# arcosoph/nanowakeword

Measured on AMD Instinct MI355X. Metric: clips/sec (1 s @16 kHz PCM->logits), higher is better.
Workload: dtype f32; 1 GPU; cnn head on (101,64) log-mel, batch=4096/GPU, 1 s 16 kHz mono int16 clips, 64-mel 25 ms/10 ms center frontend, fused STFT+mel HIP kernel, fp32; clips_per_gpu=4096, n_samples=16000, parallelism=batch-split x1

## Files before the change

### nanowakeword_amd/build.py

```python
from __future__ import annotations

import os
import shutil
import subprocess
import sys

PKG = os.path.dirname(os.path.abspath(__file__))
ROOT = os.path.dirname(PKG)
CSRC = os.path.join(PKG, "csrc")
LIB = os.path.join(PKG, "libnwwhip.so")
EMU_DIR = os.path.join(ROOT, "tests", "hostemu")
EMU_LIB = os.path.join(EMU_DIR, "libfe_emu.so")

HIP_SOURCES = ["nww_api.hip", "nww_weights.hip", "nww_plan.hip", "nww_stream.hip", "nww_comm.hip", "nww_emb.hip", "frontend2.hip", "layers.hip", "gemm_x3.hip", "trunk.hip", "trunk_b.hip", "conv3_x3.hip", "ffn_x3.hip", "lin_x3.hip", "dual_x3.hip", "bc_chain.hip", "rnn_x3.hip", "rnn_stream.hip", "mha_mfma.hip", "mha_h2.hip", "attn_x3.hip", "emb_stream.hip", "tcn_x3.hip", "merge_x3.hip", "qn_x3.hip", "raw_conv.hip", "raw_x3.hip", "fe_tables.cpp"]


def _hipcc() -> str:
    for c in (os.environ.get("HIPCC"), shutil.which("hipcc"), "/opt/rocm/bin/hipcc"):
        if c and os.path.exists(c):
            return c
    raise RuntimeError("hipcc not found")


def _newer(target: str, deps) -> bool:
    if not os.path.exists(target):
        return True
    t = os.path.getmtime(target)
    return any(os.path.getmtime(d) > t for d in deps)


NO_SLP = {"frontend2.hip", "trunk_b.hip", "dual_x3.hip", "bc_chain.hip", "layers.hip", "ffn_x3.hip"}


def build_hip(force: bool = False, verbose: bool = False, out: str = LIB) -> str:
    from concurrent.futures import ThreadPoolExecutor
    tag = "" if out == LIB else "_" + os.path.splitext(os.path.basename(out))[0]
    odir = os.path.join(PKG, "build" + tag)
    os.makedirs(odir, exist_ok=True)
    mode = os.environ.get("NWW_SLP", "")
    extra = os.environ.get("NWW_HIPCC_FLAGS", "").split()
    headers = [os.path.join(CSRC, f) for f in os.listdir(CSRC) if f.endswith(".h")] + [os.path.join(ROOT, "include", "nww.h")]
    jobs, objs = [], []
    for src in HIP_SOURCES:
        sp = os.path.join(CSRC, src)
        obj = os.path.join(odir, os.path.splitext(src)[0] + ".o")
        objs.append(obj)
        if not force and not _newer(obj, [sp] + headers):
            continue
        no_slp = mode == "none" or (mode != "all" and src in NO_SLP)
        jobs.append([_hipcc(), "--offload-arch=gfx950", "-O3", "-std=c++17", "-fPIC"] + (["-fno-slp-vectorize"] if no_slp else []) + extra +
                    ["-I", CSRC, "-I", os.path.join(ROOT, "include"), "-x", "hip", "-c", sp, "-o", obj])
    if not jobs and os.path.exists(out) and not _newer(out, objs):
        return out

    def run(cmd):
        if verbose:
            print(" ".join(cmd), flush=True)
        subprocess.run(cmd, check=True)
    with ThreadPoolExecutor(max_workers=max(1, int(os.environ.get("NWW_BUILD_JOBS", "6")))) as ex:
        list(ex.map(run, jobs))
    subprocess.run([_hipcc(), "--offload-arch=gfx950", "-shared", "-fPIC", "-o", out] + objs, check=True)
    return out


def build_emu(force: bool = False) -> str:
    srcs = [os.path.join(EMU_DIR, "fe_emu.cpp"), os.path.join(CSRC, "fe_tables.cpp")]
    deps = srcs + [os.path.join(CSRC, "fe_steps.h"), os.path.join(CSRC, "fe_tables.h")]
    if not force and not _newer(EMU_LIB, deps):
        return EMU_LIB
    subprocess.run(["g++", "-O2", "-std=c++17", "-shared", "-fPIC", "-I", CSRC, "-o", EMU_LIB] + srcs, check=True)
    return EMU_LIB


if __name__ == "__main__":
    print(build_hip(force="--force" in sys.argv, verbose=True))
    print(build_emu(force="--force" in sys.argv))
```

### nanowakeword_amd/csrc/fe_steps.h

```cpp
#pragma once
#include <math.h>
#include <stdint.h>

#if defined(__HIPCC__)
#include <hip/hip_runtime.h>
#define NWW_HD __host__ __device__ __forceinline__
typedef float2 nww_c32;
#else
#define NWW_HD inline
struct nww_c32 { float x, y; };
#endif

#define FE_NFFT 400
#define FE_M 200
#define FE_BINS 201
#define FE_PSTRIDE 209
#define FE_MAX_MELS 128
#define FE_MAX_MELW 640

NWW_HD nww_c32 c_make(float x, float y) { nww_c32 r; r.x = x; r.y = y; return r; }
NWW_HD nww_c32 c_add(nww_c32 a, nww_c32 b) { return c_make(a.x + b.x, a.y + b.y); }
NWW_HD nww_c32 c_sub(nww_c32 a, nww_c32 b) { return c_make(a.x - b.x, a.y - b.y); }
NWW_HD nww_c32 c_mul(nww_c32 a, nww_c32 b) { return c_make(a.x * b.x - a.y * b.y, a.x * b.y + a.y * b.x); }
NWW_HD nww_c32 c_mul_negi(nww_c32 a) { return c_make(a.y, -a.x); }
// ... 69 lines not shown
    for (int b = 0; b < 5; ++b) {
        if (SEQ) NWW_SCHED_FENCE();
        dft5(u[b][0], u[b][1], u[b][2], u[b][3], u[b][4]);
        if (b > 0) {
#pragma unroll
            for (int c = 1; c < 5; ++c) u[b][c] = c_mul(u[b][c], w25(b * c));
        }
    }
#pragma unroll
    for (int c = 0; c < 5; ++c) {
        if (SEQ) NWW_SCHED_FENCE();
        dft5(u[0][c], u[1][c], u[2][c], u[3][c], u[4][c]);
#pragma unroll
        for (int d = 0; d < 5; ++d) store(c + 5 * d, u[d][c]);
    }
    if (SEQ) NWW_SCHED_FENCE();
}

NWW_HD void fe_s1(int f, int n2, int hop, const int16_t* span, const FeTables* tb, nww_c32* yz) {
    const uint32_t* fr = (const uint32_t*)(span + hop * f);
    nww_c32 z[8];
#pragma unroll
    for (int n1 = 0; n1 < 8; ++n1) {
        const int m = 25 * n1 + n2;
        const nww_c32 w = tb->win2[m];
        const uint32_t v = fr[m];
        z[n1] = c_make((float)(int16_t)(v & 0xffffu) * w.x, (float)(int16_t)(v >> 16) * w.y);
    }
    dft8(z);
    nww_c32* out = yz + (f * 8) * 25 + n2;
    out[0] = z[0];
#pragma unroll
    for (int k1 = 1; k1 < 8; ++k1) out[k1 * 25] = c_mul(z[k1], tb->tw200[k1 * 25 + n2]);
}

NWW_HD void fe_s2(int f, int k1, nww_c32* yz) {
    nww_c32* row = yz + (f * 8 + k1) * 25;
    dft25([&](int i) { return row[i]; }, [&](int i, nww_c32 v) { row[i] = v; });
}

NWW_HD void fe_s3_core(nww_c32 A, nww_c32 B, nww_c32 tw, float* pa, float* pb) {
    const nww_c32 E = c_make(A.x + B.x, A.y - B.y);
    const nww_c32 O = c_make(A.y + B.y, B.x - A.x);
    const nww_c32 wO = c_mul(tw, O);
    const nww_c32 Xa = c_add(E, wO), Xb = c_sub(E, wO);
    *pa = Xa.x * Xa.x + Xa.y * Xa.y;
    *pb = Xb.x * Xb.x + Xb.y * Xb.y;
}
NWW_HD int fe_zpos(int k) { return (k & 7) * 25 + (k >> 3); }

NWW_HD void fe_s3(int f, int k, const FeTables* tb, const nww_c32* yz, float* pw) {
    const nww_c32* zf = yz + f * 200;
    const int kb = (k == 0) ? 0 : 200 - k;
    float* p = pw + f * FE_PSTRIDE;
    fe_s3_core(zf[fe_zpos(k)], zf[fe_zpos(kb)], tb->tw400[k], &p[k], &p[200 - k]);
}

NWW_HD float fe_s4(int f, int j, const FeTables* tb, const float* pw) {
    const float* p = pw + f * FE_PSTRIDE + tb->mel_lo[j];
    const float* w = tb->melw + tb->mel_off[j];
    const int n = tb->mel_cnt[j];
    float acc = 0.0f;
    for (int i = 0; i < n; ++i) acc = fmaf(p[i], w[i], acc);
    return acc;
}

NWW_HD float fe_db(float mel, float amin, float mult) {
    return mult * log10f(fmaxf(mel, amin));
}

NWW_HD int fe_reflect(int s, int N) {
    if (s < 0) s = -s;
    if (s >= N) s = 2 * (N - 1) - s;
    return s;
}

#define FE2_G 8
#define FE2_FRAME_DW 400
#define FE2_PSHIFT(f) (4 * ((f) >> 1))
#define FE2_STAGE_OFF 216
#define FE2_MAX_TILES 8
#define FE2_MAX_STEPS 512

#define FE2_CHUNK 8
#define FE2_MAX_CHUNKS 64
struct Fe2MelPlan {
    int32_t ntiles;
    int32_t total_steps;
    int32_t nchunks;
    int32_t tile_k0[FE2_MAX_TILES];
    int32_t tile_nsteps[FE2_MAX_TILES];
    int32_t tile_first[FE2_MAX_TILES];
    uint32_t chunk_meta[FE2_MAX_CHUNKS];
    float b[FE2_MAX_STEPS * 64];
};

NWW_HD void fe2_s1(const uint32_t s[8], const nww_c32 win[8], const nww_c32 tw[7], nww_c32 z[8]) {
#pragma unroll
    for (int n1 = 0; n1 < 8; ++n1)
        z[n1] = c_make((float)(int16_t)(s[n1] & 0xffffu) * win[n1].x, (float)(int16_t)(s[n1] >> 16) * win[n1].y);
    dft8(z);
#pragma unroll
    for (int k1 = 1; k1 < 8; ++k1) z[k1] = c_mul(z[k1], tw[k1 - 1]);
}

NWW_HD float fe2_mel_planned(const Fe2MelPlan* pl, const float* p, int j) {
    const int t = j >> 4, n = j & 15;
    const int k0 = pl->tile_k0[t], ns = pl->tile_nsteps[t];
    const float* b = pl->b + (size_t)pl->tile_first[t] * 64 + n;
    float acc[2] = {0.0f, 0.0f};
    for (int s = 0; s < ns; ++s)
        for (int kk = 0; kk < 4; ++kk) acc[s & 1] = fmaf(p[k0 + 4 * s + kk], b[s * 64 + kk * 16], acc[s & 1]);
    return acc[0] + acc[1];
}
```

### nanowakeword_amd/csrc/fe_tables.cpp

```cpp
#include "fe_tables.h"
#include <cmath>
#include <cstring>

static const double kPi = 3.14159265358979323846;

void fe_default_window(int win_length, std::vector<float>& window) {
    window.resize(win_length);
    for (int n = 0; n < win_length; ++n)
        window[n] = (float)(0.5 - 0.5 * std::cos(2.0 * kPi * n / win_length));
}

void fe_default_melfb(const FeParams& p, std::vector<float>& fb) {
    const int n_freqs = p.n_fft / 2 + 1;
    fb.assign((size_t)n_freqs * p.n_mels, 0.f);
    const double m_min = 2595.0 * std::log10(1.0 + (double)p.f_min / 700.0);
    const double m_max = 2595.0 * std::log10(1.0 + (double)p.f_max / 700.0);
    std::vector<double> f_pts(p.n_mels + 2);
    for (int i = 0; i < p.n_mels + 2; ++i) {
        const double m = m_min + (m_max - m_min) * i / (p.n_mels + 1);
        f_pts[i] = 700.0 * (std::pow(10.0, m / 2595.0) - 1.0);
    }
    const double nyq = (double)(p.sample_rate / 2);
    for (int k = 0; k < n_freqs; ++k) {
        const double f = nyq * k / (n_freqs - 1);
// ... 6 lines not shown
    }
}

std::string fe_build_tables(const FeParams& p, const float* window, const float* fb, FeTables* t) {
    if (p.n_fft != FE_NFFT) return "only n_fft=400 is implemented";
    if (p.win_length > p.n_fft || p.win_length <= 0) return "win_length must be in 1..n_fft";
    if (p.n_mels <= 0 || p.n_mels > FE_MAX_MELS) return "n_mels must be in 1..128";
    if (p.hop <= 0 || (p.hop & 1)) return "hop_length must be positive and even";
    std::memset(t, 0, sizeof(*t));
    std::vector<float> wp(p.n_fft, 0.f);
    const int pad_left = (p.n_fft - p.win_length) / 2;
    for (int i = 0; i < p.win_length; ++i) wp[pad_left + i] = window[i];
    for (int m = 0; m < FE_M; ++m) {
        t->win2[m].x = wp[2 * m] * (1.0f / 65536.0f);
        t->win2[m].y = wp[2 * m + 1] * (1.0f / 65536.0f);
    }
    for (int n2 = 0; n2 < 25; ++n2)
        for (int k1 = 0; k1 < 8; ++k1) {
            const double a = -2.0 * kPi * (double)(n2 * k1) / 200.0;
            t->tw200[k1 * 25 + n2].x = (float)std::cos(a);
            t->tw200[k1 * 25 + n2].y = (float)std::sin(a);
        }
    for (int k = 0; k <= 100; ++k) {
        const double a = -2.0 * kPi * (double)k / 400.0;
        t->tw400[k].x = (float)std::cos(a);
        t->tw400[k].y = (float)std::sin(a);
    }
    int off = 0;
    for (int j = 0; j < p.n_mels; ++j) {
        int lo = -1, hi = -1;
        for (int k = 0; k < FE_BINS; ++k)
            if (fb[(size_t)k * p.n_mels + j] != 0.f) { if (lo < 0) lo = k; hi = k; }
        if (lo < 0) { lo = 0; hi = -1; }
        const int cnt = hi - lo + 1;
        if (off + cnt > FE_MAX_MELW) return "mel filterbank has too many non-zeros for the LDS table";
        t->mel_lo[j] = lo; t->mel_cnt[j] = cnt; t->mel_off[j] = off;
        for (int i = 0; i < cnt; ++i) t->melw[off + i] = fb[(size_t)(lo + i) * p.n_mels + j];
        off += cnt;
    }
    return "";
}

int fe_num_frames(const FeParams& p, int n) {
    if (p.center) {
        if (n <= p.n_fft / 2) return -1;
        return 1 + n / p.hop;
    }
    if (n < p.n_fft) return -1;
    return 1 + (n - p.n_fft) / p.hop;
}

std::string fe2_build_mel_plan(const FeParams& p, const float* fb, Fe2MelPlan* pl) {
    std::memset(pl, 0, sizeof(*pl));
    const int ntiles = (p.n_mels + 15) / 16;
    if (ntiles > FE2_MAX_TILES) return "n_mels must be <= 128";
    pl->ntiles = ntiles;
    int first = 0;
    for (int t = 0; t < ntiles; ++t) {
        int lo = FE_BINS, hi = -1;
        for (int k = 0; k < FE_BINS; ++k)
            for (int n = 0; n < 16; ++n) {
                const int j = 16 * t + n;
                if (j < p.n_mels && fb[(size_t)k * p.n_mels + j] != 0.f) { if (k < lo) lo = k; if (k > hi) hi = k; }
            }
        if (hi < 0) { lo = 0; hi = 0; }
        int ns = (hi - lo + 1 + 3) / 4;
        ns = (ns + FE2_CHUNK - 1) / FE2_CHUNK * FE2_CHUNK;
        if (first + ns > FE2_MAX_STEPS || (first + ns) / FE2_CHUNK > FE2_MAX_CHUNKS) return "mel filterbank is too dense for the MFMA plan";
        for (int c = 0; c < ns / FE2_CHUNK; ++c)
            pl->chunk_meta[first / FE2_CHUNK + c] =
                (uint32_t)(lo + 4 * FE2_CHUNK * c) | ((uint32_t)t << 12) | ((c == ns / FE2_CHUNK - 1) ? 1u << 16 : 0u);
        pl->tile_k0[t] = lo; pl->tile_nsteps[t] = ns; pl->tile_first[t] = first;
        for (int s = 0; s < ns; ++s)
            for (int l = 0; l < 64; ++l) {
                const int k = lo + 4 * s + (l >> 4), j = 16 * t + (l & 15);
                pl->b[(size_t)(first + s) * 64 + l] = (k < FE_BINS && j < p.n_mels) ? fb[(size_t)k * p.n_mels + j] : 0.f;
            }
        first += ns;
    }
    pl->total_steps = first;
    pl->nchunks = first / FE2_CHUNK;
    return "";
}
```

### nanowakeword_amd/csrc/fe_tables.h

```cpp
#pragma once
#include <string>
#include <vector>
#include "fe_steps.h"

struct FeParams {
    int sample_rate = 16000, n_fft = 400, win_length = 400, hop = 160, n_mels = 64, center = 1;
    float f_min = 0.f, f_max = 8000.f, amin = 1e-10f, db_mult = 10.f;
};

void fe_default_window(int win_length, std::vector<float>& window);
void fe_default_melfb(const FeParams& p, std::vector<float>& fb);

std::string fe_build_tables(const FeParams& p, const float* window, const float* fb, FeTables* out);

std::string fe2_build_mel_plan(const FeParams& p, const float* fb, Fe2MelPlan* out);

int fe_num_frames(const FeParams& p, int n_samples);
```

### nanowakeword_amd/csrc/frontend2.hip

```cpp
#include <hip/hip_runtime.h>
#include <stdlib.h>
#include "fe_steps.h"
#include "frontend.h"
#include "layers.h"

typedef float f32x4 __attribute__((ext_vector_type(4)));

struct Fe2MelLds {
    uint32_t desc[FE_MAX_MELS];
    float w[FE_MAX_MELW];
};

__device__ __forceinline__ void fe2_wave_sync() {
    __builtin_amdgcn_fence(__ATOMIC_RELEASE, "wavefront");
    __builtin_amdgcn_wave_barrier();
    __builtin_amdgcn_fence(__ATOMIC_ACQUIRE, "wavefront");
}

__device__ __forceinline__ void fe2_load_column(const int16_t* __restrict__ x, int base, int n2, uint32_t v[8]) {
    const uint32_t* p = reinterpret_cast<const uint32_t*>(x + base) + n2;
#pragma unroll
    for (int n1 = 0; n1 < 8; ++n1) v[n1] = p[25 * n1];
}

__device__ __forceinline__ float fe2_db(float mel, float amin, float mult, float floor_db) {
    const float db = (mult * 0.30102999566398120f) * __log2f(fmaxf(mel, amin));
    return mel > amin ? db : floor_db;
}

#define FE2_PARAMS                                                                                                      \
    const int16_t *__restrict__ pcm, size_t row_stride, int B, int N, int T, int ngroups, int hop, int pad, int n_mels,    \
        float amin, float db_mult, float floor_db, const FeTables *__restrict__ gtb, const Fe2MelPlan *__restrict__ plan,  \
        float *__restrict__ out_db, float *__restrict__ out_mel, int frames_major, int dbg, int gsz, Fe2Sub sub
#define FE2_ARGS pcm, row_stride, B, N, T, ngroups, hop, pad, n_mels, amin, db_mult, floor_db, gtb, plan, out_db, out_mel, frames_major, dbg, gsz, sub
template <int MEL, int FAST_OUT, int MAXT, bool RING, bool FLAT>
__device__ __forceinline__ void fe2_wave_body(FE2_PARAMS) {
    static_assert(!FLAT || (FAST_OUT && !RING && MEL == 2), "flat items: frames-major fast output, register filters, no frame subsets");
#ifndef NWW_ABLATION
    if (FLAT) dbg = 0;
#endif
    extern __shared__ __attribute__((aligned(16))) char smem[];
    constexpr int MFMA_MEL = MEL == 1;
    const int lane = threadIdx.x & 63;
    const int wv = __builtin_amdgcn_readfirstlane((int)(threadIdx.x >> 6));
    const int nwv = blockDim.x >> 6;
    const int tb_bytes = MEL == 0 ? (int)sizeof(Fe2MelLds) : 0;
    Fe2MelLds* mt = reinterpret_cast<Fe2MelLds*>(smem);
    float* slab = reinterpret_cast<float*>(smem + tb_bytes) + wv * (FE2_G * FE2_FRAME_DW);
    if (MEL == 0) {
        for (int i = threadIdx.x; i < FE_MAX_MELS; i += blockDim.x)
            mt->desc[i] = (uint32_t)gtb->mel_lo[i] | ((uint32_t)gtb->mel_cnt[i] << 8) | ((uint32_t)gtb->mel_off[i] << 16);
        for (int i = threadIdx.x; i < FE_MAX_MELW; i += blockDim.x) mt->w[i] = gtb->melw[i];
        __syncthreads();
    }
    const int n2 = lane % 25, slot = lane / 25;
    nww_c32 win[8], tw[7];
#pragma unroll
    for (int n1 = 0; n1 < 8; ++n1) win[n1] = gtb->win2[25 * n1 + n2];
#pragma unroll
    for (int k1 = 1; k1 < 8; ++k1) tw[k1 - 1] = gtb->tw200[k1 * 25 + n2];
    const int k3a = lane, k3b = 64 + lane;
    const bool has_b = k3b <= 100;
    const nww_c32 twa = gtb->tw400[k3a], twb = gtb->tw400[has_b ? k3b : 100];
    const int ia2 = k3a ? FE_M - k3a : 0;
    const int f2 = lane >> 3, k1_2 = lane & 7;
    constexpr int NCO = FLAT ? 2 : 4;
    int co_off[NCO];
#pragma unroll
    for (int r = 0; r < NCO; ++r) {
        const int i = 4 * lane + 256 * r, f = i / n_mels, j = i - f * n_mels;
        co_off[r] = f * FE2_FRAME_DW + FE2_STAGE_OFF + FE2_PSHIFT(f) + j;
    }
    const int mel_l5 = lane & 31;
    const int mel_j = (lane & 32) + ((mel_l5 < 4) ? mel_l5 : (mel_l5 < 12) ? 12 + mel_l5 : (mel_l5 < 16) ? mel_l5 - 8 : (mel_l5 < 20) ? 8 + mel_l5
                                     : (mel_l5 < 28) ? mel_l5 - 12 : mel_l5);
    float wreg[MAXT];
    int mel_lo_lane = 0;
    if (MEL == 2) {
        const int j = min(mel_j, n_mels - 1);
        const int lo = gtb->mel_lo[j], sh4 = lo & 3;
        mel_lo_lane = lo - sh4;
        const int cnt = mel_j < n_mels ? gtb->mel_cnt[j] : 0, off = gtb->mel_off[j];
#pragma unroll
        for (int i = 0; i < MAXT; ++i) wreg[i] = (i >= sh4 && i - sh4 < cnt) ? gtb->melw[off + i - sh4] : 0.0f;
    }
    const int mel_nchunks = MFMA_MEL ? plan->nchunks : 0;
    const uint32_t mel_meta = MFMA_MEL ? plan->chunk_meta[lane] : 0u;
    const bool aligned = ((reinterpret_cast<uintptr_t>(pcm) | (row_stride * sizeof(int16_t))) & 3) == 0;

    const int total = FLAT ? (B * T + FE2_G - 1) / FE2_G : B * ngroups;
    const int stride = gridDim.x * nwv;
    uint32_t cur[8];
    auto geom = [&](int item, int& b, int& t0, int& nf) {
        b = item / ngroups;
        const int g = item - b * ngroups;
        if (!RING || sub.nr == 0) {
            t0 = g * gsz;
            nf = min(gsz, T - t0);
        } else {
            int r = 0;
            while (r + 1 < sub.nr && g >= sub.gend[r]) ++r;
            t0 = sub.t0[r] + (g - (r ? sub.gend[r - 1] : 0)) * gsz;
            nf = min(gsz, sub.t1[r] - t0);
        }
    };
    auto interior = [&](int t0, int nf) {
        const int s0 = t0 * hop - pad;
        return aligned && s0 >= 0 && s0 + (nf - 1) * hop + FE_NFFT <= N;
    };
    auto prefetch_first = [&](int item) {
        int b, t0, nf;
        geom(item, b, t0, nf);
        if (interior(t0, nf) && slot < nf && slot < 2)
            fe2_load_column(pcm + (size_t)b * row_stride, (t0 + slot) * hop - pad, n2, cur);
    };
    auto flat_frame = [&](int t0, int nf, int k, uint32_t& woff, int& s0) {
        int f = 2 * k + slot;
        if (nf < FE2_G) f = min(f, nf - 1);
        int t = t0 + f;
        woff = 0u;
        if (t0 + FE2_G > T)
            while (t >= T) { t -= T; woff += (uint32_t)row_stride; }
        s0 = t * hop - pad;
    };
    auto flat_load = [&](const int16_t* x, uint32_t woff, int s0, uint32_t (&v)[8]) {
        const bool edge = !aligned || __builtin_amdgcn_ballot_w64(s0 < 0 || s0 + FE_NFFT > N) != 0;
        const char* xb = reinterpret_cast<const char*>(x);
        if (!edge) {
            const uint32_t o = 2u * (woff + (uint32_t)s0 + 2u * (uint32_t)n2);
#pragma unroll
            for (int n1 = 0; n1 < 8; ++n1) v[n1] = *reinterpret_cast<const uint32_t*>(xb + o + 100 * n1);
        } else {
            uint32_t lo[8], hi[8];
#pragma unroll
            for (int n1 = 0; n1 < 8; ++n1) {
                const int q = s0 + 2 * (n2 + 25 * n1);
                lo[n1] = *reinterpret_cast<const uint16_t*>(xb + 2u * (woff + (uint32_t)fe_reflect(q, N)));
                hi[n1] = *reinterpret_cast<const uint16_t*>(xb + 2u * (woff + (uint32_t)fe_reflect(q + 1, N)));
            }
#pragma unroll
            for (int n1 = 0; n1 < 8; ++n1) v[n1] = lo[n1] | (hi[n1] << 16);
        }
    };
    auto flat_plain = [&](int t0, int nf) {
        const int s0 = t0 * hop - pad;
        return aligned && nf == FE2_G && t0 + FE2_G <= T && s0 >= 0 && s0 + (FE2_G - 1) * hop + FE_NFFT <= N;
    };
    auto plain_off = [&](int t0, int k) { return 2u * (uint32_t)((t0 + 2 * k + slot) * hop - pad + 2 * n2); };
    auto plain_load = [&](const int16_t* x, uint32_t o, uint32_t (&v)[8]) {
        const char* xb = reinterpret_cast<const char*>(x);
#pragma unroll
        for (int n1 = 0; n1 < 8; ++n1) v[n1] = *reinterpret_cast<const uint32_t*>(xb + o + 100 * n1);
    };
    auto flat_first = [&](const int16_t* x, int t0, int nf) {
        if (lane < 50) {
            if (flat_plain(t0, nf)) {
                plain_load(x, plain_off(t0, 0), cur);
            } else {
                uint32_t woff; int s0;
                flat_frame(t0, nf, 0, woff, s0);
                flat_load(x, woff, s0, cur);
            }
        }
    };
    int item = __builtin_amdgcn_readfirstlane((int)(blockIdx.x * nwv + wv));
    int fb = 0, ft = 0, fdb = 0, fdt = 0;
    if (FLAT) {
        const int g0 = FE2_G * item, step = FE2_G * stride;
        fb = g0 / T; ft = g0 - fb * T;
        fdb = step / T; fdt = step - fdb * T;
    }
    if (item < total) {
        if (FLAT) flat_first(pcm + (size_t)fb * row_stride, ft, min(FE2_G, B * T - FE2_G * item));
        else prefetch_first(item);
    }
    for (; item < total; item += stride) {
        int b, t0, nf;
        if (FLAT) { b = fb; t0 = ft; nf = min(FE2_G, B * T - FE2_G * item); }
        else geom(item, b, t0, nf);
        const int16_t* x = pcm + (size_t)b * row_stride;
        if (FLAT) {
            auto s1_trip = [&](int f) {
                if (!(dbg & 1)) {
                    nww_c32 z[8];
                    fe2_s1(cur, win, tw, z);
                    nww_c32* y = reinterpret_cast<nww_c32*>(slab + f * FE2_FRAME_DW) + n2;
#pragma unroll
                    for (int k1 = 0; k1 < 8; ++k1) y[k1 * 25] = z[k1];
                }
            };
            if (lane < 50) {
                if (flat_plain(t0, nf)) {
                    uint32_t o = plain_off(t0, 1);
#pragma unroll 1
                    for (int k = 0; k < FE2_G / 2; ++k) {
                        uint32_t nxt[8];
                        plain_load(x, o, nxt);
                        s1_trip(2 * k + slot);
#pragma unroll
                        for (int n1 = 0; n1 < 8; ++n1) cur[n1] = nxt[n1];
                        if (k + 2 < FE2_G / 2) o += 4u * (uint32_t)hop;
                    }
                } else {
#pragma unroll 1
                    for (int k = 0; k < FE2_G / 2; ++k) {
                        uint32_t nxt[8];
                        uint32_t woff; int s0;
                        flat_frame(t0, nf, min(k + 1, FE2_G / 2 - 1), woff, s0);
                        flat_load(x, woff, s0, nxt);
                        s1_trip(2 * k + slot);
#pragma unroll
                        for (int n1 = 0; n1 < 8; ++n1) cur[n1] = nxt[n1];
                    }
                }
            }
        } else {
            const bool inner = interior(t0, nf);
            const uint32_t* span = reinterpret_cast<const uint32_t*>(slab + 6 * FE2_FRAME_DW);
            if (!inner) {
                const int s0 = t0 * hop - pad, npairs = ((nf - 1) * hop + FE_NFFT) >> 1;
                uint32_t* sp = reinterpret_cast<uint32_t*>(slab + 6 * FE2_FRAME_DW);
                for (int i = lane; i < npairs; i += 64) {
                    const int q = s0 + 2 * i;
                    sp[i] = (uint32_t)(uint16_t)x[fe_reflect(q, N)] | ((uint32_t)(uint16_t)x[fe_reflect(q + 1, N)] << 16);
                }
                fe2_wave_sync();
                if (slot < nf && slot < 2) {
#pragma unroll
                    for (int n1 = 0; n1 < 8; ++n1) cur[n1] = span[((slot * hop) >> 1) + n2 + 25 * n1];
                }
            }
            const int nit = (nf + 1) >> 1;
#pragma unroll 1
            for (int it = 0; it < nit; ++it) {
                const int f = 2 * it + slot, fn = f + 2;
                uint32_t nxt[8];
#pragma unroll
                for (int n1 = 0; n1 < 8; ++n1) nxt[n1] = 0u;
                if (slot < 2 && fn < nf && it + 1 < FE2_G / 2) {
                    if (inner) {
                        fe2_load_column(x, (t0 + fn) * hop - pad, n2, nxt);
                    } else {
#pragma unroll
                        for (int n1 = 0; n1 < 8; ++n1) nxt[n1] = span[((fn * hop) >> 1) + n2 + 25 * n1];
                    }
                }
                if (slot < 2 && f < nf && !(dbg & 1)) {
                    nww_c32 z[8];
                    fe2_s1(cur, win, tw, z);
                    nww_c32* y = reinterpret_cast<nww_c32*>(slab + f * FE2_FRAME_DW) + n2;
#pragma unroll
                    for (int k1 = 0; k1 < 8; ++k1) y[k1 * 25] = z[k1];
                }
#pragma unroll
                for (int n1 = 0; n1 < 8; ++n1) cur[n1] = nxt[n1];
            }
        }
        fe2_wave_sync();
        if (f2 < nf && !(dbg & 2)) {
            nww_c32* zf = reinterpret_cast<nww_c32*>(slab + f2 * FE2_FRAME_DW);
            const nww_c32* row = zf + k1_2 * 25;
            nww_c32* dst = zf + k1_2;
            dft25<true>([&](int i) { return row[i]; }, [&](int i, nww_c32 v) { dst[8 * i] = v; });
        }
        fe2_wave_sync();
        if (FLAT) {
            fb += fdb; ft += fdt;
            if (ft >= T) { ft -= T; ++fb; }
            if (item + stride < total) flat_first(pcm + (size_t)fb * row_stride, ft, min(FE2_G, B * T - FE2_G * (item + stride)));
        } else if (item + stride < total) prefetch_first(item + stride);
        if (!(dbg & 4)) {
            const nww_c32* z0 = reinterpret_cast<const nww_c32*>(slab);
            nww_c32 a1 = z0[k3a], b1 = z0[ia2], a2 = z0[has_b ? k3b : 0], b2 = z0[has_b ? FE_M - k3b : 0];
#pragma unroll
            for (int f = 0; f < FE2_G; ++f) {
                if (f >= nf) break;
                nww_c32 na1 = a1, nb1 = b1, na2 = a2, nb2 = b2;
                if (f + 1 < FE2_G) {
                    const nww_c32* zn = reinterpret_cast<const nww_c32*>(slab + (f + 1) * FE2_FRAME_DW);
                    na1 = zn[k3a]; nb1 = zn[ia2]; na2 = zn[has_b ? k3b : 0]; nb2 = zn[has_b ? FE_M - k3b : 0];
                }
                float pa1, pb1, pa2, pb2;
                fe_s3_core(a1, b1, twa, &pa1, &pb1);
                fe_s3_core(a2, b2, twb, &pa2, &pb2);
                float* p = slab + f * FE2_FRAME_DW + FE2_PSHIFT(f);
                p[k3a] = pa1;
                p[FE_M - k3a] = pb1;
                if (has_b) { p[k3b] = pa2; p[FE_M - k3b] = pb2; }
                a1 = na1; b1 = nb1; a2 = na2; b2 = nb2;
            }
        }
        fe2_wave_sync();
        if (!(dbg & 8)) {
            if (MFMA_MEL) {
                const int fa = lane & 7;
                const float* arow = slab + fa * FE2_FRAME_DW + FE2_PSHIFT(fa) + (lane >> 4);
                const float* bp = plan->b + lane;
                f32x4 acc0 = {0.f, 0.f, 0.f, 0.f}, acc1 = {0.f, 0.f, 0.f, 0.f};
                auto load_chunk = [&](int c, float (&av)[FE2_CHUNK], float (&bv)[FE2_CHUNK]) {
                    const float* ap = arow + (__builtin_amdgcn_readlane(mel_meta, c) & 0xfff);
                    const float* bq = bp + (size_t)((dbg & 16) ? 0 : c) * (FE2_CHUNK * 64);
#pragma unroll
                    for (int s = 0; s < FE2_CHUNK; ++s) { av[s] = ap[4 * s]; bv[s] = bq[64 * s]; }
                };
                auto run_chunk = [&](int c, const float (&av)[FE2_CHUNK], const float (&bv)[FE2_CHUNK]) {
#pragma unroll
                    for (int s = 0; s < FE2_CHUNK; s += 2) {
                        acc0 = __builtin_amdgcn_mfma_f32_16x16x4f32(av[s], bv[s], acc0, 0, 0, 0);
                        acc1 = __builtin_amdgcn_mfma_f32_16x16x4f32(av[s + 1], bv[s + 1], acc1, 0, 0, 0);
                    }
                    const uint32_t meta = __builtin_amdgcn_readlane(mel_meta, c);
                    if (meta & 0x10000u) {
                        const int j = 16 * ((meta >> 12) & 0xf) + (lane & 15);
                        if (lane < 32 && j < n_mels) {
                            if (FAST_OUT) {
                                float* st = slab + (4 * (lane >> 4)) * FE2_FRAME_DW + FE2_STAGE_OFF + FE2_PSHIFT(4 * (lane >> 4)) + j;
#pragma unroll
                                for (int i = 0; i < 4; ++i)
                                    st[i * FE2_FRAME_DW + FE2_PSHIFT(i)] = fe2_db(acc0[i] + acc1[i], amin, db_mult, floor_db);
                            } else {
#pragma unroll
                                for (int i = 0; i < 4; ++i) {
                                    const int f = 4 * (lane >> 4) + i;
                                    const float m = acc0[i] + acc1[i];
                                    const float db = fe2_db(m, amin, db_mult, floor_db);
                                    if (f < nf) {
                                        if (frames_major) {
                                            slab[f * FE2_FRAME_DW + FE2_STAGE_OFF + FE2_PSHIFT(f) + j] = db;
                                            if (out_mel) out_mel[((size_t)b * T + t0 + f) * n_mels + j] = m;
                                        } else {
                                            const size_t o = ((size_t)b * n_mels + j) * T + t0 + f;
                                            if (out_db) out_db[o] = db;
                                            if (out_mel) out_mel[o] = m;
                                        }
                                    }
                                }
                            }
                        }
                        acc0 = f32x4{0.f, 0.f, 0.f, 0.f};
                        acc1 = f32x4{0.f, 0.f, 0.f, 0.f};
                    }
                };
                float a0[FE2_CHUNK], b0[FE2_CHUNK], a1[FE2_CHUNK], b1[FE2_CHUNK];
                const int last = mel_nchunks - 1;
                load_chunk(0, a0, b0);
#pragma unroll 1
                for (int c = 0; c < mel_nchunks; c += 2) {
                    load_chunk(min(c + 1, last), a1, b1);
                    run_chunk(c, a0, b0);
                    load_chunk(min(c + 2, last), a0, b0);
                    if (c + 1 < mel_nchunks) run_chunk(c + 1, a1, b1);
                }
// ... 74 lines not shown
                    *reinterpret_cast<float4*>(base + (size_t)(x < sub.ring_rows ? x + sub.ring_rows : x - sub.ring_rows) * n_mels + j) = v;
                }
            } else {
            float* dst = out_db + ((size_t)b * T + t0) * n_mels;
            if ((n_mels & 3) == 0) {
#pragma unroll
                for (int r = 0; r < NCO; ++r) {
                    const int i = 4 * lane + 256 * r;
                    if (i < cnt) *reinterpret_cast<float4*>(dst + i) = *reinterpret_cast<const float4*>(slab + co_off[r]);
                }
            } else {
                for (int i = lane; i < cnt; i += 64) {
                    const int f = i / n_mels, j = i - f * n_mels;
                    dst[i] = slab[f * FE2_FRAME_DW + FE2_STAGE_OFF + FE2_PSHIFT(f) + j];
                }
            }
            }
        }
        fe2_wave_sync();
    }
}

template <int MEL, int FAST_OUT, int MAXT, bool RING = false, bool FLAT = false>
__global__ void __launch_bounds__(256, 3) fe2_wave_kernel(FE2_PARAMS) { fe2_wave_body<MEL, FAST_OUT, MAXT, RING, FLAT>(FE2_ARGS); }

bool fe2_subset_supported(const FeParams& p, int mel_mode) { return mel_mode != 0 && (p.n_mels & 3) == 0; }

int fe2_lds_bytes(int waves, int mel_mode) {
    return waves * FE2_G * FE2_FRAME_DW * 4 + (mel_mode == 0 ? (int)sizeof(Fe2MelLds) : 0);
}

hipError_t fe2_launch(const int16_t* d_pcm, size_t row_stride, int B, int N, int T, const FeParams& p,
                      const FeTables* d_tables, const Fe2MelPlan* d_plan, float* d_db, float* d_mel, int frames_major,
                      int mel_mode, int max_taps, int block, int max_grid, hipStream_t stream, const Fe2Sub* subset) {
    if (block < 64 || block > 1024 || (block & 63)) return hipErrorInvalidValue;
    const int nwv = block / 64;
    Fe2Sub sub = subset ? *subset : Fe2Sub{};
    if (sub.nr < 0 || sub.nr > 4) return hipErrorInvalidValue;
    if ((sub.nr || sub.ring_rows) && !(frames_major && d_db && !d_mel && (p.n_mels & 3) == 0)) return hipErrorInvalidValue;
    if (sub.ring_rows && (sub.ring_rows < T || sub.row0 < 0 || sub.row0 >= sub.ring_rows)) return hipErrorInvalidValue;
    auto count_groups = [&](int g) {
        if (sub.nr == 0) return (T + g - 1) / g;
        int n = 0;
        for (int r = 0; r < sub.nr; ++r) { n += (sub.t1[r] - sub.t0[r] + g - 1) / g; sub.gend[r] = n; }
        return n;
    };
    for (int r = 0; r < sub.nr; ++r)
        if (sub.t0[r] < 0 || sub.t1[r] <= sub.t0[r] || sub.t1[r] > T) return hipErrorInvalidValue;
    int ngroups = count_groups(FE2_G);
    int mode = mel_mode;
    if (mode == 2 && (p.n_mels > 64 || max_taps > 25)) mode = 1;
    const int lds = fe2_lds_bytes(nwv, mode);
    const int fast = (frames_major && d_db && !d_mel) ? 1 : 0;
    const bool ring = sub.nr > 0 || sub.ring_rows > 0;
    if (ring && (mode == 0 || !fast)) return hipErrorInvalidValue;
#ifdef NWW_ABLATION
    static const int dbg = [] { const char* e = getenv("NWW_FE_DBG"); return e ? atoi(e) : 0; }();
#else
    const int dbg = 0;
#endif
    const int small_g = 2;
    int gsz = FE2_G;
    if (mode == 2 && small_g >= 2 && small_g < FE2_G && (small_g % 2) == 0 && (long long)B * ngroups * 4 <= (long long)max_grid * nwv) {
        gsz = small_g;
        ngroups = count_groups(gsz);
    }
    const bool flat = fast && !ring && mode == 2 && gsz == FE2_G && T != FE2_G && (long long)B * T <= 0x7fffffffLL - FE2_G &&
                      (unsigned long long)row_stride * FE2_G + (unsigned long long)N < (1ull << 31);
    auto kern = mode == 0 ? fe2_wave_kernel<0, 0, 1>
              : mode == 1 ? (ring ? fe2_wave_kernel<1, 1, 1, true> : fast ? fe2_wave_kernel<1, 1, 1> : fe2_wave_kernel<1, 0, 1>)
              : max_taps <= 17 ? (ring ? fe2_wave_kernel<2, 1, 20, true> : flat ? fe2_wave_kernel<2, 1, 20, false, true> : fast ? fe2_wave_kernel<2, 1, 20> : fe2_wave_kernel<2, 0, 20>)
                               : (ring ? fe2_wave_kernel<2, 1, 28, true> : flat ? fe2_wave_kernel<2, 1, 28, false, true> : fast ? fe2_wave_kernel<2, 1, 28> : fe2_wave_kernel<2, 0, 28>);
    const void* fn = reinterpret_cast<const void*>(kern);
    {
        hipError_t e = nww_allow_lds(fn, (size_t)lds);
        if (e != hipSuccess) return e;
    }
    const long long total = flat ? ((long long)B * T + FE2_G - 1) / FE2_G : (long long)B * ngroups;
    long long need = (total + nwv - 1) / nwv;
    int grid = (int)(need < max_grid ? need : max_grid);
    if (grid < 1) grid = 1;
    const int pad = p.center ? FE_NFFT / 2 : 0;
    hipLaunchKernelGGL(kern, dim3(grid), dim3(block), lds, stream, d_pcm, row_stride, B, N, T, ngroups, p.hop, pad, p.n_mels,
                       p.amin, p.db_mult, p.db_mult * log10f(p.amin), d_tables, d_plan, d_db, d_mel, frames_major, dbg, gsz, sub);
    return hipGetLastError();
}
```

### nanowakeword_amd/csrc/nww_weights.hip

```cpp
#include "nww_internal.h"

namespace {
using Shape = std::vector<int64_t>;
struct SpecBuilder {
    std::vector<std::string>& keys;
    std::map<std::string, HostTensor>& t;
    void add(const std::string& k, Shape s) { keys.push_back(k); t[k].shape = std::move(s); }
    void lin(const std::string& p, int out, int in) { add(p + ".weight", {out, in}); add(p + ".bias", {out}); }
    void ln(const std::string& p, int d) { add(p + ".weight", {d}); add(p + ".bias", {d}); }
    void bn(const std::string& p, int c) {
        add(p + ".weight", {c}); add(p + ".bias", {c}); add(p + ".running_mean", {c}); add(p + ".running_var", {c});
    }
    void gru(const std::string& p, int in, int H, int layers, int G = 3) {
        for (int l = 0; l < layers; ++l) {
            const int isz = l == 0 ? in : 2 * H;
            for (const char* sfx : {"", "_reverse"}) {
                const std::string s = "_l" + std::to_string(l) + sfx;
                add(p + ".weight_ih" + s, {G * H, isz}); add(p + ".weight_hh" + s, {G * H, H});
                add(p + ".bias_ih" + s, {G * H}); add(p + ".bias_hh" + s, {G * H});
            }
        }
    }
};

// ... 242 lines not shown
            }
            tb.data[co] = (float)bias;
        }
        tdw.shape = {k, Cp}; tdw.data.assign((size_t)k * Cp, 0.0f);
        double amax = 0.0;
        for (int ci = 0; ci < Cin; ++ci) {
            double sum = 0.0;
            for (int j = 0; j < k; ++j) { tdw.data[(size_t)j * Cp + ci] = dw[(size_t)ci * k + j]; sum += std::fabs((double)dw[(size_t)ci * k + j]); }
            amax = std::fmax(amax, sum);
        }
        tam.shape = {1}; tam.data = {(float)(amax * (1.0 + 1e-6))};
        for (auto* t : {&tpw, &tres, &tb, &tdw, &tam, &tcat}) t->loaded = !t->data.empty();
        h->tensors[p + ".qn.pw"] = tpw; h->tensors[p + ".qn.bias"] = tb; h->tensors[p + ".qn.dw_t"] = tdw; h->tensors[p + ".qn.amax"] = tam;
        if (proj) h->tensors[p + ".qn.res"] = tres;
        if (cat) h->tensors[p + ".qn.wcat"] = tcat;
    }
}

void fold_raw_frontend(nww_handle* h) {
    const nww_config& c = h->cfg;
    for (int i = 0, Cin = 1; i < c.n_blocks; ++i) {
        const int Cout = c.layer_dim << i, k = i == 0 ? 41 : 13;
        const std::string conv = "model.frontend.conv_blocks." + std::to_string(3 * i), bn = "model.frontend.conv_blocks." + std::to_string(3 * i + 1);
        const auto &w = h->tensors[conv + ".weight"].data, &g = h->tensors[bn + ".weight"].data, &b = h->tensors[bn + ".bias"].data,
                   &mu = h->tensors[bn + ".running_mean"].data, &var = h->tensors[bn + ".running_var"].data;
        HostTensor tw, tb;
        tw.shape = {k, Cin, Cout}; tw.data.resize((size_t)k * Cin * Cout);
        tb.shape = {Cout}; tb.data.resize(Cout);
        for (int co = 0; co < Cout; ++co) {
            const double al = (double)g[co] / std::sqrt((double)var[co] + 1e-5);
            tb.data[co] = (float)((double)b[co] - (double)mu[co] * al);
            for (int ci = 0; ci < Cin; ++ci)
                for (int j = 0; j < k; ++j) tw.data[((size_t)j * Cin + ci) * Cout + co] = (float)(al * (double)w[((size_t)co * Cin + ci) * k + j]);
        }
        tw.loaded = tb.loaded = true;
        h->tensors[conv + ".raw.w"] = tw; h->tensors[conv + ".raw.b"] = tb;
        if (i > 0 && Cout % 32 == 0 && Cin % 16 == 0) {
            HostTensor tk;
            tk.shape = {Cout, k * Cin}; tk.data.resize((size_t)Cout * k * Cin);
            for (int co = 0; co < Cout; ++co)
                for (int j = 0; j < k; ++j)
                    for (int ci = 0; ci < Cin; ++ci) tk.data[((size_t)co * k + j) * Cin + ci] = tw.data[((size_t)j * Cin + ci) * Cout + co];
            tk.loaded = true;
            h->tensors[conv + ".raw.wk"] = tk;
        }
        Cin = Cout;
    }
}

int upload_weight_arena(nww_handle* h) {
    size_t total = 0;
    for (auto& kv : h->tensors) {
        if (!kv.second.loaded || kv.first.rfind("frontend.", 0) == 0) continue;
        kv.second.dev_off = total;
        total += (kv.second.data.size() + 3) & ~(size_t)3;
    }
    HIP_TRY(h, hipMalloc(&h->d_weights, (total + 4) * sizeof(float)));
    for (auto& kv : h->tensors) {
        if (!kv.second.loaded || kv.first.rfind("frontend.", 0) == 0) continue;
        HIP_TRY(h, hipMemcpy(h->d_weights + kv.second.dev_off, kv.second.data.data(), kv.second.data.size() * sizeof(float),
                             hipMemcpyHostToDevice));
    }
    return NWW_OK;
}

int build_frontend_tables(nww_handle* h) {
    std::vector<float> win, fb;
    auto wi = h->tensors.find("frontend.window");
    if (wi != h->tensors.end() && wi->second.loaded) win = wi->second.data; else fe_default_window(h->fe.win_length, win);
    auto fi = h->tensors.find("frontend.mel_fb");
    if (fi != h->tensors.end() && fi->second.loaded) fb = fi->second.data; else fe_default_melfb(h->fe, fb);
    FeTables tb;
    const std::string e = fe_build_tables(h->fe, win.data(), fb.data(), &tb);
    if (!e.empty()) return fail(h, NWW_ERR_INVALID, "frontend tables: %s", e.c_str());
    const size_t tbytes = (sizeof(FeTables) + 15) & ~(size_t)15;
    HIP_TRY(h, hipMalloc(&h->d_tables, tbytes));
    HIP_TRY(h, hipMemset(h->d_tables, 0, tbytes));
    HIP_TRY(h, hipMemcpy(h->d_tables, &tb, sizeof(FeTables), hipMemcpyHostToDevice));
    h->mel_max_taps = 0;
    for (int j = 0; j < h->fe.n_mels; ++j) h->mel_max_taps = tb.mel_cnt[j] > h->mel_max_taps ? tb.mel_cnt[j] : h->mel_max_taps;
    std::vector<Fe2MelPlan> plan(1);
    const std::string e2 = fe2_build_mel_plan(h->fe, fb.data(), plan.data());
    if (!e2.empty()) return fail(h, NWW_ERR_INVALID, "frontend mel plan: %s", e2.c_str());
    HIP_TRY(h, hipMalloc(&h->d_melplan, sizeof(Fe2MelPlan)));
    HIP_TRY(h, hipMemcpy(h->d_melplan, plan.data(), sizeof(Fe2MelPlan), hipMemcpyHostToDevice));
    return NWW_OK;
}
```

Before: 9.063 million clips/s.

## Precompute per-lane mel weights and prefetch-touch next flat item's PCM span

Builds a per-lane mel filter table on the host so each lane loads its register filter weights as contiguous float4 reads, replacing per-tap gathers and branching. In flat mode, each lane also issues a dummy 16-bit load spread across the next item's PCM span, pinned with an asm barrier, to warm the cache ahead of use. The wave count is now passed as a kernel argument instead of being derived from blockDim. This adds extra loads and a larger plan struct, plus a host test library build.

Measured after the change: 9.109 million clips/s, median of 6. About the same (+0.5%).

```diff
diff --git a/nanowakeword_amd/build.py b/nanowakeword_amd/build.py
--- a/nanowakeword_amd/build.py
+++ b/nanowakeword_amd/build.py
@@ -11,6 +11,7 @@
 LIB = os.path.join(PKG, "libnwwhip.so")
 EMU_DIR = os.path.join(ROOT, "tests", "hostemu")
 EMU_LIB = os.path.join(EMU_DIR, "libfe_emu.so")
+TOUCH_LIB = os.path.join(EMU_DIR, "libfe_touch.so")
 
 HIP_SOURCES = ["nww_api.hip", "nww_weights.hip", "nww_plan.hip", "nww_stream.hip", "nww_comm.hip", "nww_emb.hip", "frontend2.hip", "layers.hip", "gemm_x3.hip", "trunk.hip", "trunk_b.hip", "conv3_x3.hip", "ffn_x3.hip", "lin_x3.hip", "dual_x3.hip", "bc_chain.hip", "rnn_x3.hip", "rnn_stream.hip", "mha_mfma.hip", "mha_h2.hip", "attn_x3.hip", "emb_stream.hip", "tcn_x3.hip", "merge_x3.hip", "qn_x3.hip", "raw_conv.hip", "raw_x3.hip", "fe_tables.cpp"]
 
@@ -63,13 +64,22 @@
     return out
 
 
+def _build_host(lib: str, source: str, force: bool) -> str:
+    srcs = [os.path.join(EMU_DIR, source), os.path.join(CSRC, "fe_tables.cpp")]
+    deps = srcs + [os.path.join(CSRC, "fe_steps.h"), os.path.join(CSRC, "fe_tables.h")]
+    if not force and not _newer(lib, deps):
+        return lib
+    subprocess.run(["g++", "-O2", "-std=c++17", "-shared", "-fPIC", "-I", CSRC, "-o", lib] + srcs, check=True)
+    return lib
+
+
 def build_emu(force: bool = False) -> str:
-    srcs = [os.path.join(EMU_DIR, "fe_emu.cpp"), os.path.join(CSRC, "fe_tables.cpp")]
-    deps = srcs + [os.path.join(CSRC, "fe_steps.h"), os.path.join(CSRC, "fe_tables.h")]
-    if not force and not _newer(EMU_LIB, deps):
-        return EMU_LIB
-    subprocess.run(["g++", "-O2", "-std=c++17", "-shared", "-fPIC", "-I", CSRC, "-o", EMU_LIB] + srcs, check=True)
-    return EMU_LIB
+    build_touch(force)
+    return _build_host(EMU_LIB, "fe_emu.cpp", force)
+
+
+def build_touch(force: bool = False) -> str:
+    return _build_host(TOUCH_LIB, "fe_touch.cpp", force)
 
 
 if __name__ == "__main__":
diff --git a/nanowakeword_amd/csrc/fe_steps.h b/nanowakeword_amd/csrc/fe_steps.h
--- a/nanowakeword_amd/csrc/fe_steps.h
+++ b/nanowakeword_amd/csrc/fe_steps.h
@@ -175,6 +175,16 @@
 #define FE2_MAX_TILES 8
 #define FE2_MAX_STEPS 512
 
+#define FE2_MAXT 28
+struct alignas(16) Fe2LaneTab {
+    float w[FE2_MAXT / 4][64][4];
+    int32_t lo[64];
+};
+NWW_HD int fe2_mel_lane_filter(int lane) {
+    const int l5 = lane & 31;
+    return (lane & 32) + ((l5 < 4) ? l5 : (l5 < 12) ? 12 + l5 : (l5 < 16) ? l5 - 8 : (l5 < 20) ? 8 + l5 : (l5 < 28) ? l5 - 12 : l5);
+}
+
 #define FE2_CHUNK 8
 #define FE2_MAX_CHUNKS 64
 struct Fe2MelPlan {
@@ -186,7 +196,20 @@
     int32_t tile_first[FE2_MAX_TILES];
     uint32_t chunk_meta[FE2_MAX_CHUNKS];
     float b[FE2_MAX_STEPS * 64];
+    Fe2LaneTab lanes;
 };
+
+NWW_HD int fe2_touch_lanes(int hop) {
+    const int n = (2 * ((FE2_G - 1) * hop + FE_NFFT) + 127) / 128 + 1;
+    return n < 64 ? n : 64;
+}
+NWW_HD int64_t fe2_touch_base(int64_t clip_first, int s0) { return 2 * (clip_first + (int64_t)s0); }
+NWW_HD uint32_t fe2_touch_rel(int64_t base, int64_t batch_samples, int lane) {
+    const int64_t room = 2 * batch_samples - 2 - base;
+    const int lo = base < 0 ? (int)-base : 0, hi = room < 8192 ? (int)room : 8192;
+    const int r = 128 * lane;
+    return (uint32_t)(r < lo ? lo : r > hi ? hi : r);
+}
 
 NWW_HD void fe2_s1(const uint32_t s[8], const nww_c32 win[8], const nww_c32 tw[7], nww_c32 z[8]) {
 #pragma unroll
diff --git a/nanowakeword_amd/csrc/fe_tables.cpp b/nanowakeword_amd/csrc/fe_tables.cpp
--- a/nanowakeword_amd/csrc/fe_tables.cpp
+++ b/nanowakeword_amd/csrc/fe_tables.cpp
@@ -112,3 +112,16 @@
     pl->nchunks = first / FE2_CHUNK;
     return "";
 }
+
+void fe2_build_lane_table(const FeParams& p, const FeTables& t, Fe2MelPlan* pl) {
+    Fe2LaneTab& lt = pl->lanes;
+    std::memset(&lt, 0, sizeof(lt));
+    for (int lane = 0; lane < 64; ++lane) {
+        const int mel_j = fe2_mel_lane_filter(lane);
+        const int j = mel_j < p.n_mels - 1 ? mel_j : p.n_mels - 1;
+        const int lo = t.mel_lo[j], sh4 = lo & 3;
+        lt.lo[lane] = lo - sh4;
+        const int cnt = mel_j < p.n_mels ? t.mel_cnt[j] : 0, off = t.mel_off[j];
+        for (int i = 0; i < FE2_MAXT; ++i) lt.w[i >> 2][lane][i & 3] = (i >= sh4 && i - sh4 < cnt) ? t.melw[off + i - sh4] : 0.0f;
+    }
+}
diff --git a/nanowakeword_amd/csrc/fe_tables.h b/nanowakeword_amd/csrc/fe_tables.h
--- a/nanowakeword_amd/csrc/fe_tables.h
+++ b/nanowakeword_amd/csrc/fe_tables.h
@@ -15,4 +15,6 @@
 
 std::string fe2_build_mel_plan(const FeParams& p, const float* fb, Fe2MelPlan* out);
 
+void fe2_build_lane_table(const FeParams& p, const FeTables& t, Fe2MelPlan* out);
+
 int fe_num_frames(const FeParams& p, int n_samples);
diff --git a/nanowakeword_amd/csrc/frontend2.hip b/nanowakeword_amd/csrc/frontend2.hip
--- a/nanowakeword_amd/csrc/frontend2.hip
+++ b/nanowakeword_amd/csrc/frontend2.hip
@@ -31,8 +31,8 @@
 #define FE2_PARAMS                                                                                                      \
     const int16_t *__restrict__ pcm, size_t row_stride, int B, int N, int T, int ngroups, int hop, int pad, int n_mels,    \
         float amin, float db_mult, float floor_db, const FeTables *__restrict__ gtb, const Fe2MelPlan *__restrict__ plan,  \
-        float *__restrict__ out_db, float *__restrict__ out_mel, int frames_major, int dbg, int gsz, Fe2Sub sub
-#define FE2_ARGS pcm, row_stride, B, N, T, ngroups, hop, pad, n_mels, amin, db_mult, floor_db, gtb, plan, out_db, out_mel, frames_major, dbg, gsz, sub
+        float *__restrict__ out_db, float *__restrict__ out_mel, int frames_major, int dbg, int gsz, int nwv, Fe2Sub sub
+#define FE2_ARGS pcm, row_stride, B, N, T, ngroups, hop, pad, n_mels, amin, db_mult, floor_db, gtb, plan, out_db, out_mel, frames_major, dbg, gsz, nwv, sub
 template <int MEL, int FAST_OUT, int MAXT, bool RING, bool FLAT>
 __device__ __forceinline__ void fe2_wave_body(FE2_PARAMS) {
     static_assert(!FLAT || (FAST_OUT && !RING && MEL == 2), "flat items: frames-major fast output, register filters, no frame subsets");
@@ -41,9 +41,9 @@
 #endif
     extern __shared__ __attribute__((aligned(16))) char smem[];
     constexpr int MFMA_MEL = MEL == 1;
+    constexpr bool TOUCH = FLAT;
     const int lane = threadIdx.x & 63;
     const int wv = __builtin_amdgcn_readfirstlane((int)(threadIdx.x >> 6));
-    const int nwv = blockDim.x >> 6;
     const int tb_bytes = MEL == 0 ? (int)sizeof(Fe2MelLds) : 0;
     Fe2MelLds* mt = reinterpret_cast<Fe2MelLds*>(smem);
     float* slab = reinterpret_cast<float*>(smem + tb_bytes) + wv * (FE2_G * FE2_FRAME_DW);
@@ -71,18 +71,17 @@
         const int i = 4 * lane + 256 * r, f = i / n_mels, j = i - f * n_mels;
         co_off[r] = f * FE2_FRAME_DW + FE2_STAGE_OFF + FE2_PSHIFT(f) + j;
     }
-    const int mel_l5 = lane & 31;
-    const int mel_j = (lane & 32) + ((mel_l5 < 4) ? mel_l5 : (mel_l5 < 12) ? 12 + mel_l5 : (mel_l5 < 16) ? mel_l5 - 8 : (mel_l5 < 20) ? 8 + mel_l5
-                                     : (mel_l5 < 28) ? mel_l5 - 12 : mel_l5);
+    const int mel_j = fe2_mel_lane_filter(lane);
     float wreg[MAXT];
     int mel_lo_lane = 0;
-    if (MEL == 2) {
-        const int j = min(mel_j, n_mels - 1);
-        const int lo = gtb->mel_lo[j], sh4 = lo & 3;
-        mel_lo_lane = lo - sh4;
-        const int cnt = mel_j < n_mels ? gtb->mel_cnt[j] : 0, off = gtb->mel_off[j];
-#pragma unroll
-        for (int i = 0; i < MAXT; ++i) wreg[i] = (i >= sh4 && i - sh4 < cnt) ? gtb->melw[off + i - sh4] : 0.0f;
+    if constexpr (MEL == 2) {
+        static_assert(MAXT % 4 == 0 && MAXT <= FE2_MAXT, "whole 16-byte pieces of the lane table");
+#pragma unroll
+        for (int i = 0; i < MAXT; i += 4) {
+            const float4 w4 = *reinterpret_cast<const float4*>(plan->lanes.w[i >> 2][lane]);
+            wreg[i] = w4.x; wreg[i + 1] = w4.y; wreg[i + 2] = w4.z; wreg[i + 3] = w4.w;
+        }
+        mel_lo_lane = plan->lanes.lo[lane];
     }
     const int mel_nchunks = MFMA_MEL ? plan->nchunks : 0;
     const uint32_t mel_meta = MFMA_MEL ? plan->chunk_meta[lane] : 0u;
@@ -163,6 +162,14 @@
             }
         }
     };
+    uint32_t touch = 0u;
+    const int touch_n = TOUCH ? fe2_touch_lanes(hop) : 0;
+    const int64_t batch_samples = (int64_t)(B - 1) * (int64_t)row_stride + N;
+    auto flat_touch = [&](int b, int t0) {
+        const int64_t base = fe2_touch_base((int64_t)b * (int64_t)row_stride, t0 * hop - pad);
+        if (lane < touch_n)
+            touch = *reinterpret_cast<const uint16_t*>(reinterpret_cast<const char*>(pcm) + base + fe2_touch_rel(base, batch_samples, lane));
+    };
     int item = __builtin_amdgcn_readfirstlane((int)(blockIdx.x * nwv + wv));
     int fb = 0, ft = 0, fdb = 0, fdt = 0;
     if (FLAT) {
@@ -171,8 +178,10 @@
         fdb = step / T; fdt = step - fdb * T;
     }
     if (item < total) {
-        if (FLAT) flat_first(pcm + (size_t)fb * row_stride, ft, min(FE2_G, B * T - FE2_G * item));
-        else prefetch_first(item);
+        if (FLAT) {
+            flat_first(pcm + (size_t)fb * row_stride, ft, min(FE2_G, B * T - FE2_G * item));
+            if (TOUCH) flat_touch(fb, ft);
+        } else prefetch_first(item);
     }
     for (; item < total; item += stride) {
         int b, t0, nf;
@@ -189,6 +198,7 @@
                     for (int k1 = 0; k1 < 8; ++k1) y[k1 * 25] = z[k1];
                 }
             };
+            if (TOUCH) asm volatile("" ::"v"(touch));
             if (lane < 50) {
                 if (flat_plain(t0, nf)) {
                     uint32_t o = plain_off(t0, 1);
@@ -267,7 +277,10 @@
         if (FLAT) {
             fb += fdb; ft += fdt;
             if (ft >= T) { ft -= T; ++fb; }
-            if (item + stride < total) flat_first(pcm + (size_t)fb * row_stride, ft, min(FE2_G, B * T - FE2_G * (item + stride)));
+            if (item + stride < total) {
+                flat_first(pcm + (size_t)fb * row_stride, ft, min(FE2_G, B * T - FE2_G * (item + stride)));
+                if (TOUCH) flat_touch(fb, ft);
+            }
         } else if (item + stride < total) prefetch_first(item + stride);
         if (!(dbg & 4)) {
             const nww_c32* z0 = reinterpret_cast<const nww_c32*>(slab);
@@ -508,6 +521,6 @@
     if (grid < 1) grid = 1;
     const int pad = p.center ? FE_NFFT / 2 : 0;
     hipLaunchKernelGGL(kern, dim3(grid), dim3(block), lds, stream, d_pcm, row_stride, B, N, T, ngroups, p.hop, pad, p.n_mels,
-                       p.amin, p.db_mult, p.db_mult * log10f(p.amin), d_tables, d_plan, d_db, d_mel, frames_major, dbg, gsz, sub);
+                       p.amin, p.db_mult, p.db_mult * log10f(p.amin), d_tables, d_plan, d_db, d_mel, frames_major, dbg, gsz, nwv, sub);
     return hipGetLastError();
 }
diff --git a/nanowakeword_amd/csrc/nww_weights.hip b/nanowakeword_amd/csrc/nww_weights.hip
--- a/nanowakeword_amd/csrc/nww_weights.hip
+++ b/nanowakeword_amd/csrc/nww_weights.hip
@@ -348,6 +348,7 @@
     std::vector<Fe2MelPlan> plan(1);
     const std::string e2 = fe2_build_mel_plan(h->fe, fb.data(), plan.data());
     if (!e2.empty()) return fail(h, NWW_ERR_INVALID, "frontend mel plan: %s", e2.c_str());
+    fe2_build_lane_table(h->fe, tb, plan.data());
     HIP_TRY(h, hipMalloc(&h->d_melplan, sizeof(Fe2MelPlan)));
     HIP_TRY(h, hipMemcpy(h->d_melplan, plan.data(), sizeof(Fe2MelPlan), hipMemcpyHostToDevice));
     return NWW_OK;
```
